# bistoyek21-ric/StrikeForce

Measured on AMD Instinct MI355X. Metric: env-steps/sec (whole node), 64x64 map x32 entities, higher is better.
Workload: dtype int32

## Files before the change

__graft_entry__.py:

```python
import os
import subprocess
import sys

ROOT = os.path.dirname(os.path.abspath(__file__))
for p in (ROOT, os.path.join(ROOT, "tests")):
    if p not in sys.path:
        sys.path.insert(0, p)


def build():
    from strikeforce_amd import build as b
    b.build()
    subprocess.check_call(["make", "-s", "-C", os.path.join(ROOT, "oracle"), "libsf_oracle.so"])
    subprocess.check_call(["make", "-s", "-C", os.path.join(ROOT, "oracle"), "ref"])
    subprocess.check_call(["make", "-s", "-C", os.path.join(ROOT, "tests", "emu"), "libsf_emu.so"])
    subprocess.check_call(["make", "-s", "-C", os.path.join(ROOT, "tests", "fixed_shape_emu"), "libsf_emu_fixed.so"])
    subprocess.check_call([sys.executable, "-B", os.path.join(ROOT, "tests", "obs_flavour.py")], stdout=subprocess.DEVNULL)
    import strikeforce_amd
    from strikeforce_amd import env
    lib = env.load_library()
    from strikeforce_amd import policy
    missing = [n for n in env.EXPORTS + policy.EXPORTS if not hasattr(lib, n)]
    if missing:
        raise RuntimeError("libstrikeforce_amd.so lacks %s" % missing)


def smoke():
    import numpy as np
    from oracle_lib import ArenaDump, Oracle, diff_dumps
    from strikeforce_amd import config, env

    w = config.baseline_workload("C1", arenas=4, device=0)
    o, g = Oracle(w), env.ArenaBatch(w)
    tb, sr = w.seeds()
    o.reset(tb, sr), g.reset(tb, sr)
    cmds, _ = config.bench_commands(4, 1, 40)
    for s in range(40):
        o.step(cmds[s]), g.step(cmds[s])
    for a in range(4):
        d = diff_dumps(o.dump(a).as_dict(), ArenaDump(*g.dump_raw(a)).as_dict())
        if d:
            raise AssertionError("smoke: arena %d differs from the oracle: %s" % (a, d))
    x, y = o.observe(), g.observe()
    ulp = np.abs(x.view(np.int32).astype(np.int64) - y.view(np.int32).astype(np.int64)).max()
    if ulp > 1:
        raise AssertionError("smoke: observation differs by %d ulp" % ulp)
    print("smoke ok: 4 arenas x 40 steps bit-exact, observation max ulp diff %d" % ulp)
    import ctypes as C
    import json
    import ref_cases
    gold = json.load(open(os.path.join(ROOT, "tests", "golden", "ref_traj.json")))["cases"]["C1"]
    wr = ref_cases.GOLDEN_CASES["C1"][0]()
    gr = env.ArenaBatch(wr)
    gr.reset((C.c_uint64 * 1)(gold["tb"]), (C.c_uint64 * 1)(gold["serial"]))
    rc, _ = config.bench_commands(1, 1, 60, seed0=gold["command_seed"])
    for s in range(60):
        if "%016x" % int(gr.digest()[0]) != gold["digests"][s]:
            raise AssertionError("smoke: state after %d steps differs from the reference's own" % s)
        gr.step(rc[s])
    print("smoke ok: 60 steps of configs[0] reproduce the reference's own per-step digests")
    import torch
    sys.path.insert(0, os.path.join(ROOT, "oracle"))
    import policy_ref
    from strikeforce_amd import policy
    params = policy.init_parameters(seed=1)
    pb = policy.PolicyBatch(params, 4)
    d_obs = torch.from_numpy(y.reshape(4, 32, 31, 31)).cuda()
    d_probs = torch.zeros((4, 9), device="cuda")
    d_value = torch.zeros(4, device="cuda")
    pb.forward(d_obs.data_ptr(), 4, d_probs.data_ptr(), d_value.data_ptr())
    pb.synchronize()
    h0 = np.zeros((2, 4, 160), dtype=np.float32)
    a0 = np.eye(9, dtype=np.float32)[[0] * 4]
    probs, value, _ = policy_ref.forward_batched(params, y.reshape(4, 32, 31, 31), h0, a0)
    err = float(np.max(np.abs(d_probs.cpu().numpy() - probs) / probs))
    if err > 5e-5 or np.max(np.abs(d_value.cpu().numpy() - value)) > 5e-5:
        raise AssertionError("smoke: policy network differs from the reference by %.3g" % err)
    print("smoke ok: policy forward for 4 agents, max relative error %.2g" % err)


if __name__ == "__main__":
    build()
    if "--smoke" in sys.argv:
        smoke()
```

strikeforce_amd/csrc/sf_api.hip:

```cpp
#include <hip/hip_runtime.h>

#include <dlfcn.h>

#include <cstddef>

#include <new>
#include <utility>
#include <vector>

#include "wave_gfx950.hpp"
#include "sf_core.hpp"
#include "sf_obs.hpp"
#include "sf_obs_kernels.hpp"
#include "sf_host.hpp"

namespace sf {

#ifdef SF_DIAG_STAMPS
__device__ uint32_t sf_diag_buffer[16 * 65536];
__device__ unsigned long long sf_diag_times[4 * 65536];
#endif

template <int NB, bool HP, bool BM, bool ZL>
__global__ __launch_bounds__(64) void k_reset(Params p, const uint64_t *tb, const uint64_t *serial) {
  extern __shared__ __attribute__((aligned(2048))) uint8_t lds[];
  Core<WaveGfx950, NB, HP, BM, ZL>::reset_body(lds, p, (int)blockIdx.x, tb, serial);
}

template <int NB, bool HP, bool BM, bool ZL, bool LOG>
__global__ __launch_bounds__(64) void k_step(Params p, const uint8_t *cmds, int k) {
  extern __shared__ __attribute__((aligned(2048))) uint8_t lds[];
  const int a = p.perm ? (int)gptr(p.perm)[blockIdx.x] : (int)blockIdx.x;
#ifdef SF_DIAG_STAMPS
  if (threadIdx.x == 0) sf_diag_times[4 * blockIdx.x] = __builtin_amdgcn_s_memrealtime();
#endif
  Core<WaveGfx950, NB, HP, BM, ZL>::template step_body_t<LOG>(lds, p, a, cmds, k);
#ifdef SF_DIAG_STAMPS
  __builtin_amdgcn_s_waitcnt(0);
  if (threadIdx.x == 0) sf_diag_times[4 * blockIdx.x + 3] = __builtin_amdgcn_s_memrealtime();
#endif
}

template <class SH>
__global__ __launch_bounds__(64) void k_step_fixed(Params p, const uint8_t *cmds, int k) {
  extern __shared__ __attribute__((aligned(2048))) uint8_t lds[];
  const int a = p.perm ? (int)gptr(p.perm)[blockIdx.x] : (int)blockIdx.x;
#ifdef SF_DIAG_STAMPS
  if (threadIdx.x == 0) sf_diag_times[4 * blockIdx.x] = __builtin_amdgcn_s_memrealtime();
#endif
  Core<WaveGfx950, SH::NB, false, true, false, SH>::template step_body_t<false>(lds, p, a, cmds, k);
#ifdef SF_DIAG_STAMPS
  __builtin_amdgcn_s_waitcnt(0);
  if (threadIdx.x == 0) sf_diag_times[4 * blockIdx.x + 3] = __builtin_amdgcn_s_memrealtime();
#endif
}

__global__ __launch_bounds__(1024) void k_rank(Params p, uint32_t *perm) {
  __shared__ uint32_t hist[72];
  const int t = (int)threadIdx.x;
  if (t < 72) hist[t] = 0u;
  __syncthreads();
  auto cls_of = [&](int a) {
    const uint32_t n = (uint32_t)gptr(p.scal)[(size_t)a * SC_WORDS + SC_LOAD];
    return 64u - (n > 64u ? 64u : n);
  };
  for (int a = t; a < p.A; a += 1024) atomicAdd(&hist[cls_of(a)], 1u);
  __syncthreads();
  if (t == 0) {
    uint32_t run = 0;
    for (int c = 0; c < 65; ++c) {
      const uint32_t n = hist[c];
      hist[c] = run;
      run += n;
    }
  }
  __syncthreads();
  for (int a = t; a < p.A; a += 1024) {
    uint32_t pos = atomicAdd(&hist[cls_of(a)], 1u);
    if ((pos >> 10) & 1u) {
      const uint32_t base = pos & ~1023u, len = (uint32_t)p.A - base < 1024u ? (uint32_t)p.A - base : 1024u;
      pos = base + (len - 1u - (pos - base));
    }
    gptr(perm)[pos] = (uint32_t)a;
  }
}

template <int NB, bool HP, bool BM, bool ZL>
__global__ __launch_bounds__(64) void k_step_half(Params p, const uint8_t *cmds, int phase) {
  extern __shared__ __attribute__((aligned(2048))) uint8_t lds[];
  Core<WaveGfx950, NB, HP, BM, ZL>::step_half_body(lds, p, (int)blockIdx.x, cmds, phase);
}

__global__ void k_agent_alive(Params p, uint8_t *out) {
  const int i = (int)(blockIdx.x * blockDim.x + threadIdx.x);
  if (i >= p.A * p.n_agents) return;
  const int a = i / p.n_agents, g = i % p.n_agents;
  const uint32_t fl = gptr(p.hum)[((size_t)HW_FLAGS * (size_t)p.A + (size_t)a) * (size_t)p.H + (size_t)g];
  gptr(out)[i] = (uint8_t)((fl & (HF_ALIVE | HF_CTRL)) == (HF_ALIVE | HF_CTRL));
}

__global__ void k_done(Params p, uint8_t *out) {
  const int i = (int)(blockIdx.x * blockDim.x + threadIdx.x);
  if (i >= p.A * p.n_agents) return;
  const SF_GLOBAL int32_t *sc = gptr(p.scal) + (size_t)(i / p.n_agents) * SC_WORDS;
  gptr(out)[i] = (uint8_t)(p.auto_reset ? sc[SC_ENDED] : sc[SC_DONE]);
}

__global__ __launch_bounds__(64) void k_ep_late(Params p, int after_reset) {
  Core<WaveGfx950, 1>::ep_log_late(p, (int)blockIdx.x, after_reset != 0);
}

__global__ __launch_bounds__(64) void k_replay_fetch(Params p, Replay r, int mode) {
  Core<WaveGfx950, 1>::replay_fetch(p, r, (int)blockIdx.x, mode);
}

__global__ __launch_bounds__(1024) void k_ep_plan(const int32_t *scal, int32_t *cursor, int A, int depth, int max_records,
                                                  int32_t *plan, int32_t *counts) {
  __shared__ int wsum[16];
  __shared__ int lost_sum;
  const int t = (int)threadIdx.x, lane = t & 63, w = t >> 6;
  const int chunk = (A + 1023) / 1024;
  const int a0 = min(t * chunk, A), a1 = min(a0 + chunk, A);
  int kept = 0, lost = 0;
#pragma unroll 4
  for (int a = a0; a < a1; ++a) {
    const int pend = max(gptr(scal)[(size_t)a * SC_WORDS + SC_EPISODES] - gptr(cursor)[a], 0);
    kept += min(pend, depth), lost += pend - min(pend, depth);
  }
  const int x = wave_scan_incl(kept, lane);
#pragma unroll
  for (int d = 32; d; d >>= 1) lost += __shfl_xor(lost, d, 64);
  if (t == 0) lost_sum = 0;
  if (lane == 63) wsum[w] = x;
// ... 587 lines not shown
```

strikeforce_amd/csrc/sf_core.hpp:

```cpp
#pragma once
#include "../../include/strikeforce.h"
#include "sf_types.hpp"

#if defined(SF_EXP_FAKE_DRAWS) && !defined(SF_EXPERIMENT_BUILD)
#error "SF_EXP_FAKE_DRAWS makes draw() return wrong numbers on purpose (tools/experiments/r03_rows): timing builds only, together with -DSF_EXPERIMENT_BUILD"
#endif

namespace sf {

enum { SH_WALL, SH_HUMAN, SH_ZOMBIE, SH_PUP, SH_PDN, SH_BULLET, SH_CHEST, SH_POUT, SH_EMPTY };
enum { LIM_PORTAL = 1000, LIM_BLOCK = 1100 };

#define SF_SHAPE(f) (SH::FIXED ? SH::f(p) : p.f)
template <class W, int NB, bool HBM_PLANE = false, bool BITMAPS = !HBM_PLANE, bool ZL = false, class SH = RuntimeShape>
struct Core {
  using V = typename W::V;
  using P = typename W::P;

  struct Arena {
    V hpos, hfl, hhp, hst, hmd, hk, hdm, hef, hc01, hc23, ht01, ht23, hbpk, hcmd;
    V zpos, zhp, zmd;
    uint32_t *zl;
    uint32_t zcap;
    uint32_t zwn;
    uint32_t zwhi;
    uint32_t *pl;
    uint32_t pwn, pwhi;
    V ba[NB], bd[NB], bb[NB], bc[NB];
    V ppos;
    V rl, rus, rseed;
    V rl2, rseed2;
    uint32_t warm;
    uint32_t wrate;
    const uint32_t *xt;
    const uint32_t *ht;
    uint32_t *bm;
    V la;
    V la2;
    uint32_t la2_ok;
    int32_t frame, kills, tkills, loot, chests, steps, episodes, done, outcome, ended;
    uint32_t jomle;
    uint32_t tb_lo, tb_hi, sr_lo, sr_hi;
    uint32_t dirty;
    uint32_t pd01, pd23, pd45;
#ifdef SF_DIAG_STAMPS
    V dacc;
    uint32_t dlast;
#endif
  };

  static constexpr uint32_t RL_ZERO = 0x10000u;
  static SF_DEV V mod65537_v(V x) {
    const V t = (x & 0xffffu) - (x >> 16);
    return W::minu(t, t + 65537u);
  }
  static SF_DEV V pow3_v(const uint32_t *xt, V m, P pred) {
    return mod65537_v(W::lds_u32(xt, m & 255u, pred) * W::lds_u32(xt + 256, m >> 8, pred));
  }

  template <bool WANT_OUT>
  static SF_DEV V draw_core(V &rl, const V &rus, const V &rseed, uint32_t &jomle, const uint32_t *xt, const Params &p) {
    const P tap = W::ltu(W::lane(), 18u) & ((rl & RL_ZERO) == 0u);
    const V pw = pow3_v(xt, (rl * rseed) & 0xffffu, tap);
    const V sum = W::sum18_row1(W::select(tap, rus * pw, V(0u))) + 1u;
    V t = mod65537_v(sum);
    t = W::select(t == 0u, V(1u), t);
    jomle += 1u;
    const uint32_t e = jomle & 0xffffu;
    const V lg = W::gload_u16(p.logt, t + (uint32_t)LOGT_OFF, W::all());
    const V lnew = (lg * e) & 0xffffu;
    rl = W::select(W::lane() == 17u, lnew, W::shl1(rl));
    if (WANT_OUT) return pow3_v(xt, lnew, W::all()) & 1023u;
    return V(0u);
  }
  static constexpr uint32_t SUM_BIAS_LANE = 63489u + 11u * 65537u;
  static_assert((32ull * SUM_BIAS_LANE) % 65537ull == 1ull, "the lanes' bias must add up to the generator's +1");
  static_assert(SUM_BIAS_LANE % 2u == 0u, "it is also a byte offset into a table of 16-bit entries");
  static_assert(16ull * SUM_BIAS_LANE > 16ull * 10ull * 65536ull, "a row's partial sum must stay positive");
  static_assert((32ull * SUM_BIAS_LANE + 18ull * 10ull * 65535ull) >> 16 < (unsigned long long)LOGT_OFF, "index below the table");
  static SF_DEV const uint16_t *log_base(const Params &p) { return p.logt + LOGT_OFF - (int)(SUM_BIAS_LANE / 2u); }
  static SF_DEV V issue_offset(const uint32_t *xt, V rl, V rseed, V rus, V &d) {
    const V m = W::mul24(rl, rseed);
    const V pr = W::pow_bytes(xt, m);
    d = (pr & 0xffffu) - (pr >> 16);
    return W::rng_reduce(d, rus, V(SUM_BIAS_LANE));
  }
  static SF_DEV uint32_t draw_issue(Arena &S, const Params &p) {
    V d;
    S.la = W::gload_u16_at(log_base(p), issue_offset(S.xt, S.rl, S.rseed, S.rus, d));
    W::rng_prio_end();
    const int32_t o = (int32_t)W::readlane(d, 18u);
    return (uint32_t)(o + ((o >> 31) & 65537)) & 1023u;
  }
  static SF_DEV uint32_t draw(Arena &S, const uint8_t *, const Params &p) {
#ifdef SF_EXP_FAKE_DRAWS
    S.jomle = S.jomle * 1664525u + 1013904223u;
    return (W::readlane(S.rl, (S.jomle >> 26) & 31u) ^ (S.jomle >> 16)) & 1023u;
#endif
    SF_PROF(PH_RNG);
    S.jomle += 1u;
    if constexpr (W::FUSED_ROUND) {
      uint32_t out;
      const V off = W::rng_round(S.rl, S.jomle, S.la, S.rseed, S.rus, V(SUM_BIAS_LANE), S.xt, out);
      S.la = W::gload_u16_at(log_base(p), off);
      return out;
    }
    S.rl = W::rng_commit(S.rl, S.jomle, S.la);
    return draw_issue(S, p);
  }

  static SF_DEV void seed_digits(V &digits, uint64_t x, uint32_t lane18 = 0u) {
    digits = V(0u);
    W::setlane(digits, 18u, lane18);
    for (int i = 0; i < 18; ++i) {
      W::setlane(digits, (uint32_t)i, (uint32_t)(x % 10u) + 1u);
      x /= 10u;
    }
  }
  static SF_DEV void srand_(Arena &S, const uint8_t *lds, const Params &p, uint64_t tb, uint64_t us) {
    S.rl = V(RL_ZERO);
    seed_digits(S.rus, us);
    seed_digits(S.rseed, tb, 1u);
    S.jomle = 18u;
    (void)lds;
    for (int i = 0; i < 1024; ++i) draw_core<false>(S.rl, S.rus, S.rseed, S.jomle, S.xt, p);
    draw_issue(S, p);
  }
  static SF_DEV void prewarm_issue(Arena &S, const Params &p) {
    V d;
    S.la2 = W::gload_u16_at(log_base(p), issue_offset(S.xt, S.rl2, S.rseed2, S.rus, d));
    S.la2_ok = 1u;
  }
// ... 1397 lines not shown
    }
    if (!W::uload_i32(sc + SC_ENDED)) return;
    const uint32_t ep = (uint32_t)W::uload_i32(sc + SC_EPISODES) - 1u;
    uint64_t tb = ((uint64_t)(uint32_t)W::uload_i32(sc + SC_TB_HI) << 32) | (uint32_t)W::uload_i32(sc + SC_TB_LO);
    if (SF_SHAPE(auto_reset)) tb -= (uint64_t)(uint32_t)p.reseed;
    const uint32_t *res = (const uint32_t *)p.results + (size_t)a * (size_t)SF_SHAPE(n_agents) * 8u;
    const uint32_t frame = (uint32_t)W::uload_i32((const int32_t *)res + 6), outcome = (uint32_t)W::uload_i32((const int32_t *)res + 7);
    V h = V((uint32_t)a);
    W::setlane(h, 1u, ep);
    W::setlane(h, 2u, (uint32_t)tb), W::setlane(h, 3u, (uint32_t)(tb >> 32));
    W::setlane(h, 4u, (uint32_t)W::uload_i32(sc + SC_SR_LO)), W::setlane(h, 5u, (uint32_t)W::uload_i32(sc + SC_SR_HI));
    W::setlane(h, 6u, (frame - 1u) / 2u), W::setlane(h, 7u, outcome);
    const V r = V(((uint32_t)a * depth + (ep & (depth - 1u))) * rw);
    W::gstore(ring, r + W::lane(), h, W::ltu(W::lane(), (uint32_t)EP_HDR_WORDS));
    const uint32_t n = 8u * (uint32_t)SF_SHAPE(n_agents);
    for (uint32_t i = 0u; i < n; i += 64u) {
      const P in = W::ltu(W::lane() + i, n);
      W::gstore(ring, r + (uint32_t)EP_HDR_WORDS + W::lane() + i, W::gload(res, W::lane() + i, in), in);
    }
  }

  static SF_DEV void replay_fetch(const Params &p, const Replay &r, int a, int mode) {
    int32_t *const st = r.status + (size_t)a * RP_WORDS;
    int32_t *const sc = p.scal + (size_t)a * SC_WORDS;
    const int32_t state = W::uload_i32(st + RP_STATE);
    const uint32_t cur = (uint32_t)W::uload_i32(st + RP_CURSOR);
    const uint32_t o0 = (uint32_t)W::uload_i32((const int32_t *)r.off + a), o1 = (uint32_t)W::uload_i32((const int32_t *)r.off + a + 1);
    const uint32_t len = o1 - o0;
    const int32_t done = W::uload_i32(sc + SC_DONE);
    const P ag = W::ltu(W::lane(), (uint32_t)SF_SHAPE(n_agents));
    const V row = W::lane() + (uint32_t)a * (uint32_t)SF_SHAPE(n_agents);
    const P me = W::lane() == (uint32_t)SF_SHAPE(ind);
    if (mode == 0) {
      bool go = false;
      if (state == SF_REPLAY_RUNNING && done) {
        W::ustore_i32(st + RP_STATE, SF_REPLAY_GAME_ENDED);
      } else if ((state == SF_REPLAY_RUNNING || state == SF_REPLAY_TRUNCATED) && !done) {
        if (state == SF_REPLAY_TRUNCATED || cur == len) {
          W::ustore_i32(sc + SC_DONE, 1), W::ustore_i32(sc + SC_OUTCOME, SF_SAMPLE_END);
          if (state == SF_REPLAY_RUNNING) W::ustore_i32(st + RP_STATE, SF_REPLAY_SAMPLE_ENDED);
        } else {
          go = true;
        }
      }
      const P first = go ? me : W::frombits(0ull);
      const V tok = W::gload_u8(r.streams, V(o0 + cur), first);
      W::gstore_u8(r.cmd, row, W::select(first, tok, V((uint32_t)'+')), ag);
      W::gstore_u8(r.taken, row, tok, ag);
      if (go) {
        W::ustore_i32(st + RP_CURSOR, (int32_t)(cur + 1u));
        W::ustore_i32(st + RP_ITER, W::uload_i32(st + RP_ITER) + 1);
      }
      return;
    }
    if (state != SF_REPLAY_RUNNING || done) return;
    const V fl = W::gload(p.hum, W::lane() + ((uint32_t)HW_FLAGS * (uint32_t)p.A + (uint32_t)a) * (uint32_t)SF_SHAPE(H), ag);
    const P takes = ag & !me & ((fl & (HF_ALIVE | HF_CTRL)) == (HF_ALIVE | HF_CTRL));
    const uint64_t bal = W::ballot(takes);
    const V line = V(cur) + W::rank_below(bal);
    const P have = takes & W::ltu(line, V(len));
    const V tok = W::gload_u8(r.streams, line + o0, have);
    W::gstore_u8(r.cmd, row, tok, have);
    W::gstore_u8(r.taken, row, tok, have);
    const uint32_t want = (uint32_t)W::popc64(bal), left = len - cur, got = want < left ? want : left;
    W::ustore_i32(st + RP_CURSOR, (int32_t)(cur + got));
    if (got < want) W::ustore_i32(st + RP_STATE, SF_REPLAY_TRUNCATED);
  }

  template <bool LOG = false>
  static SF_DEV void loop_top(Arena &S, uint8_t *lds, const Params &p, int a) {
    SF_PROF(PH_TOP);
    spawns(S, lds, p);
    const int out = check_end(S, p);
    if (out != SF_RUNNING) {
      S.done = 1, S.outcome = out;
      latch_results<LOG>(S, p, a);
    }
  }

  static SF_DEV void reset_state(Arena &S, uint8_t *lds, const Params &p, uint64_t tb, uint64_t serial, bool adopt) {
    S.frame = S.kills = S.tkills = S.loot = S.chests = S.steps = 0;
    S.done = 0, S.outcome = SF_RUNNING;
    S.tb_lo = (uint32_t)tb, S.tb_hi = (uint32_t)(tb >> 32), S.sr_lo = (uint32_t)serial, S.sr_hi = (uint32_t)(serial >> 32);
    S.hpos = V(POS_NONE), S.hfl = V(0u), S.hhp = V(0u), S.hst = V(0u), S.hmd = V(0u), S.hk = V(0u), S.hdm = V(0u);
    S.hef = V(0u), S.hc01 = V(0u), S.hc23 = V(0u), S.ht01 = V(0u), S.ht23 = V(0u), S.hbpk = V(0u);
    S.hcmd = V((uint32_t)'+');
    S.zpos = V(0u), S.zhp = V(0u), S.zmd = V(0u);
    if constexpr (ZL) S.zwn = 0u;
#pragma unroll
    for (int j = 0; j < NB; ++j) S.ba[j] = V(0u), S.bd[j] = V(0u), S.bb[j] = V(0u), S.bc[j] = V(0u);
    if constexpr (ZL) {
      S.ppos = V(0u);
      S.pwn = (uint32_t)p.pw0;
      for (uint32_t j = 0; j < S.pwn; ++j) {
        const V sl = W::lane() + 64u * j;
        W::lds_store_u32(S.pl + 64u * j, W::lane(), W::gload(p.map_exits, sl, W::ltu(sl, (uint32_t)p.P)), W::all());
      }
      if (S.pwhi < S.pwn) S.pwhi = S.pwn;
    } else {
      S.ppos = W::gload(p.map_exits, W::lane(), W::ltu(W::lane(), (uint32_t)p.P));
    }
    W::copy_g2l(lds, p.map_flags, (uint32_t)SF_SHAPE(cells_pad));
    S.dirty = 1u;
    if (adopt) {
      prewarm(S, lds, p, 1024u);
      S.rl = S.rl2, S.rseed = S.rseed2, S.jomle = 18u + 1024u;
      draw_issue(S, p);
    } else {
      srand_(S, lds, p, tb, serial);
    }
    if (SF_SHAPE(auto_reset)) {
      seed_digits(S.rseed2, tb + (uint64_t)(uint32_t)p.reseed, 1u);
      S.rl2 = V(RL_ZERO);
      S.warm = 0u, S.la2_ok = 0u;
    }
    const int count = SF_SHAPE(mode) == SF_MODE_BATTLE ? SF_SHAPE(n_agents) : (SF_SHAPE(mode) == SF_MODE_SQUAD ? 10 : 1);
    SF_NOUNROLL for (int i = 0; i < count; ++i) {
      int prof = 0, team = 1;
      uint32_t q = pos_pack(0, 1, 1), fl = HF_CTRL;
      if (SF_SHAPE(mode) == SF_MODE_BATTLE) {
        q = POS_NONE, team = p.tab->teams[i], fl = HF_CTRL | (i != SF_SHAPE(ind) ? HF_REMOTE : 0u);
      } else if (SF_SHAPE(mode) == SF_MODE_SQUAD) {
        prof = i ? 1 : 0;
        team = i < 5 ? 1 : 2;
        q = i == 0 ? pos_pack(0, 3, 1) : pos_pack(i < 5 ? 0 : p.squad_floor, 1, i + 1);
        fl = (i == 0 || i < SF_SHAPE(n_agents)) ? HF_CTRL : 0u;
      }
      human_make(S, p, (uint32_t)i, prof, q, 1, team, fl, (SF_SHAPE(mode) == SF_MODE_BATTLE && p.npc_block > 1) ? i : 0);
    }
    if (SF_SHAPE(mode) == SF_MODE_BATTLE) {
      S.hfl = S.hfl & ~HF_OCC;
      SF_NOUNROLL for (int i = 0; i < SF_SHAPE(n_agents); ++i) {
        const uint32_t way = draw(S, lds, p) % 4u + 1u;
        SF_NOUNROLL for (int guard = 0; guard < (1 << 20); ++guard) {
          const uint32_t q = draw_cell(S, lds, p);
          uint32_t fl;
          if (showit_q(S, lds, p, q, fl) == SH_EMPTY) {
            W::setlane(S.hpos, (uint32_t)i, q);
            W::setlane(S.hfl, (uint32_t)i, ((W::readlane(S.hfl, (uint32_t)i) & ~HF_WAY_MASK) | way) | HF_OCC);
            break;
          }
        }
      }
    }
  }

  template <int PHASE = 0, bool LOG = false>
  static SF_DEV void step(Arena &S, uint8_t *lds, const Params &p, int a) {
    if (S.done) return;
    SF_STAMP(S, 0);
    uint32_t rest = 0u;
    SF_NOUNROLL for (int half = (PHASE == 2 ? 1 : 0); half < (PHASE == 1 ? 1 : 2); ++half) {
      const uint32_t j0 = S.jomle;
      if (half == 0) {
        zombie_action(S, lds, p);
        SF_STAMP(S, 1);
      } else {
        human_action(S, lds, p, a);
        SF_STAMP(S, 3);
      }
      const uint32_t j1 = S.jomle;
      if (half == 0) {
        portal_damage(S, lds, p);
        SF_STAMP(S, 2);
      }
      if (SF_SHAPE(auto_reset)) prewarm(S, lds, p, S.wrate);
      SF_STAMP(S, 4);
      update_tmp(S, lds, p, a);
      SF_STAMP(S, 5);
      hits(S, p);
      SF_STAMP(S, 6);
      ++S.frame;
      if (SF_SHAPE(auto_reset)) prewarm(S, lds, p, S.wrate);
      SF_STAMP(S, 4);
      const uint32_t j2 = S.jomle;
      update_bull(S, lds, p);
      SF_STAMP(S, 7);
      const uint32_t w = ((j1 - j0) & 0xffffu) | ((S.jomle - j2) << 16);
      rest += j2 - j1;
      if (half == 0)
        S.pd01 = w;
      else
        S.pd23 = w;
    }
    if (PHASE == 1) return;
    ++S.steps;
    SF_NOUNROLL for (int pass = 0; pass < 2; ++pass) {
      const uint32_t j3 = S.jomle;
      loop_top<LOG>(S, lds, p, a);
      if (pass == 0) S.pd45 = ((S.jomle - j3) & 0xffffu) | (rest << 16);
      if (!S.done || pass == 1) break;
      if (S.ended < 255) ++S.ended;
      ++S.episodes;
      if (!SF_SHAPE(auto_reset)) break;
      const uint64_t tb = (((uint64_t)S.tb_hi << 32) | S.tb_lo) + (uint64_t)(uint32_t)p.reseed;
      const uint64_t sr = ((uint64_t)S.sr_hi << 32) | S.sr_lo;
      const int32_t ep = S.episodes;
      reset_state(S, lds, p, tb, sr, true);
      S.episodes = ep;
      ++S.frame;
    }
    SF_STAMP(S, 8);
  }

  static SF_DEV void load(Arena &S, uint8_t *lds, const Params &p, int a, bool copy_plane = true) {
    const V ln = W::lane();
    const size_t AH = (size_t)p.A * (size_t)SF_SHAPE(H), AZ = (size_t)p.A * (size_t)SF_SHAPE(Z), AB = (size_t)p.A * (size_t)SF_SHAPE(B);
    {
      const P in = W::ltu(ln, (uint32_t)SF_SHAPE(H));
      const uint32_t *h = p.hum + (size_t)a * (size_t)SF_SHAPE(H);
      S.hpos = W::gload(h + HW_POS * AH, ln, in), S.hfl = W::gload(h + HW_FLAGS * AH, ln, in);
      S.hhp = W::gload(h + HW_HP * AH, ln, in), S.hst = W::gload(h + HW_STAMINA * AH, ln, in);
      S.hmd = W::gload(h + HW_MINDAMAGE * AH, ln, in), S.hk = W::gload(h + HW_KILLS * AH, ln, in);
      S.hdm = W::gload(h + HW_DAMAGE * AH, ln, in), S.hef = W::gload(h + HW_EFFECT * AH, ln, in);
      S.hc01 = W::gload(h + HW_CONS01 * AH, ln, in), S.hc23 = W::gload(h + HW_CONS23 * AH, ln, in);
      S.ht01 = W::gload(h + HW_THR01 * AH, ln, in), S.ht23 = W::gload(h + HW_THR23 * AH, ln, in);
      S.hbpk = W::gload(h + HW_BPK * AH, ln, in);
      S.hcmd = V((uint32_t)'+');
    }
    if constexpr (ZL) {
      S.zpos = V(0u), S.zhp = V(0u), S.zmd = V(0u);
      const uint32_t *z = p.zom + (size_t)a * (size_t)SF_SHAPE(Z);
      S.zwn = (uint32_t)W::uload_i32(p.scal + (size_t)a * SC_WORDS + SC_ZWN);
      if (S.zwn > (uint32_t)zw_for(SF_SHAPE(Z))) S.zwn = (uint32_t)zw_for(SF_SHAPE(Z));
      S.zwhi = S.zwn;
      for (uint32_t j = 0; j < S.zwn; ++j) {
        const V sl = ln + 64u * j;
        const P in = W::ltu(sl, (uint32_t)SF_SHAPE(Z));
        zl_put(S, ZW_POS, j, W::gload(z + ZW_POS * AZ, sl, in), W::all());
        zl_put(S, ZW_HP, j, W::gload(z + ZW_HP * AZ, sl, in), W::all());
        zl_put(S, ZW_MINDAMAGE, j, W::gload(z + ZW_MINDAMAGE * AZ, sl, in), W::all());
      }
    } else {
      const P in = W::ltu(ln, (uint32_t)SF_SHAPE(Z));
      const uint32_t *z = p.zom + (size_t)a * (size_t)SF_SHAPE(Z);
      S.zpos = W::gload(z + ZW_POS * AZ, ln, in), S.zhp = W::gload(z + ZW_HP * AZ, ln, in);
      S.zmd = W::gload(z + ZW_MINDAMAGE * AZ, ln, in);
    }
#pragma unroll
    for (int j = 0; j < NB; ++j) {
      const V sl = ln + (uint32_t)(64 * j);
      const P in = W::ltu(sl, (uint32_t)SF_SHAPE(B));
      const uint32_t *b = p.bul + (size_t)a * (size_t)SF_SHAPE(B);
      S.ba[j] = W::gload(b + BW_A * AB, sl, in), S.bd[j] = W::gload(b + BW_DAMAGE * AB, sl, in);
      S.bb[j] = W::gload(b + BW_B * AB, sl, in), S.bc[j] = W::gload(b + BW_C * AB, sl, in);
    }
    if constexpr (ZL) {
      S.ppos = V(0u);
      S.pwn = (uint32_t)W::uload_i32(p.scal + (size_t)a * SC_WORDS + SC_PWN);
      if (S.pwn > (uint32_t)zw_for(p.P)) S.pwn = (uint32_t)zw_for(p.P);
      S.pwhi = S.pwn;
      for (uint32_t j = 0; j < S.pwn; ++j) {
        const V sl = ln + 64u * j;
        W::lds_store_u32(S.pl + 64u * j, ln, W::gload(p.por + (size_t)a * (size_t)p.P, sl, W::ltu(sl, (uint32_t)p.P)), W::all());
      }
    } else {
      S.ppos = W::gload(p.por + (size_t)a * (size_t)p.P, ln, W::ltu(ln, (uint32_t)p.P));
    }
    {
      const P in = W::ltu(ln, 18u);
      const V rw = W::gload(p.rng + (size_t)a * RNG_WORDS, ln, in);
      const V val = rw & 0xfffffu;
      S.rus = (rw >> 20) & 15u, S.rseed = W::select(ln == 18u, V(1u), (rw >> 24) & 15u);
        const P nz = in & (val != 0u);
      S.rl = W::select(nz, W::gload_u16(p.logt, val + (uint32_t)LOGT_OFF, nz), V(RL_ZERO));
      const V rw2 = W::gload(p.rng2 + (size_t)a * RNG_WORDS, ln, in);
      S.rl2 = rw2 & 0x1ffffu, S.rseed2 = W::select(ln == 18u, V(1u), rw2 >> 24);
    }
    const V sc = W::gload((const uint32_t *)p.scal + (size_t)a * SC_WORDS, ln, W::ltu(ln, (uint32_t)SC_WORDS));
    S.frame = (int32_t)W::readlane(sc, SC_FRAME), S.kills = (int32_t)W::readlane(sc, SC_KILLS);
    S.tkills = (int32_t)W::readlane(sc, SC_TKILLS), S.loot = (int32_t)W::readlane(sc, SC_LOOT);
    S.chests = (int32_t)W::readlane(sc, SC_CHESTS), S.jomle = W::readlane(sc, SC_JOMLE);
    S.steps = (int32_t)W::readlane(sc, SC_STEPS), S.episodes = (int32_t)W::readlane(sc, SC_EPISODES);
    S.done = (int32_t)W::readlane(sc, SC_DONE), S.outcome = (int32_t)W::readlane(sc, SC_OUTCOME);
    S.ended = (int32_t)W::readlane(sc, SC_ENDED);
    S.tb_lo = W::readlane(sc, SC_TB_LO), S.tb_hi = W::readlane(sc, SC_TB_HI);
    S.sr_lo = W::readlane(sc, SC_SR_LO), S.sr_hi = W::readlane(sc, SC_SR_HI);
    S.warm = W::readlane(sc, SC_WARM);
    S.pd01 = W::readlane(sc, SC_PD01), S.pd23 = W::readlane(sc, SC_PD23), S.pd45 = W::readlane(sc, SC_PD45);
    if (!HBM_PLANE && copy_plane) W::copy_g2l(lds, p.flags + (size_t)a * (size_t)SF_SHAPE(cells_pad), (uint32_t)SF_SHAPE(cells_pad));
    S.dirty = 0u;
    if (copy_plane) draw_issue(S, p);
  }

  static SF_DEV void store(const Arena &S, const uint8_t *lds, const Params &p, int a) {
// ... 72 lines not shown
      W::setlane(sc, SC_LOAD, (uint32_t)(W::popc64(W::ballot(((S.zpos & ZF_ALIVE) != 0u) & W::ltu(ln, (uint32_t)SF_SHAPE(Z)))) +
                                         W::popc64(W::ballot(((S.hfl & HF_ALIVE) != 0u) & W::ltu(ln, (uint32_t)SF_SHAPE(H))))));
    }
    W::gstore((uint32_t *)p.scal + (size_t)a * SC_WORDS, ln, sc, W::ltu(ln, (uint32_t)SC_WORDS));
    if (!HBM_PLANE && S.dirty) W::copy_l2g(p.flags + (size_t)a * (size_t)SF_SHAPE(cells_pad), lds, (uint32_t)SF_SHAPE(cells_pad));
  }

  static SF_DEV uint8_t *tables(Arena &S, uint8_t *lds, const Params &p, int a, bool copy = true) {
    uint8_t *tab = lds;
    if (copy) {
      W::copy_g2l(tab, reinterpret_cast<const uint8_t *>(p.exptab), (uint32_t)LDS_EXP_BYTES);
      W::copy_g2l(tab + LDS_EXP_BYTES, reinterpret_cast<const uint8_t *>(p.tab->hatab), (uint32_t)p.ht_bytes);
    }
    S.xt = reinterpret_cast<const uint32_t *>(tab);
    S.ht = reinterpret_cast<const uint32_t *>(tab + LDS_EXP_BYTES);
    S.bm = nullptr;
    if (BITMAPS) {
      S.bm = reinterpret_cast<uint32_t *>(lds + p.lds_tab + (HBM_PLANE ? 0 : SF_SHAPE(cells_pad)));
      W::lds_zero(S.bm, (uint32_t)(BM_COUNT * SF_SHAPE(bm_words)));
    }
    S.zl = nullptr, S.zcap = 0u, S.zwn = 0u, S.zwhi = 0u;
    S.pl = nullptr, S.pwn = 0u, S.pwhi = 0u;
    if constexpr (ZL) {
      S.zl = reinterpret_cast<uint32_t *>(lds + p.lds_tab + (HBM_PLANE ? 0 : SF_SHAPE(cells_pad)) + (BITMAPS ? BM_COUNT * 4 * SF_SHAPE(bm_words) : 0));
      S.zcap = 64u * (uint32_t)zw_for(SF_SHAPE(Z));
      S.pl = S.zl + ZW_WORDS * S.zcap;
    }
    S.la = V(0u);
    S.la2 = V(0u), S.la2_ok = 0u;
    return HBM_PLANE ? p.flags + (size_t)a * (size_t)SF_SHAPE(cells_pad) : lds + p.lds_tab;
  }

  static SF_DEV void reset_body(uint8_t *lds, const Params &p, int a, const uint64_t *tb, const uint64_t *serial) {
    Arena S;
    S.episodes = 0, S.ended = 0;
    S.pd01 = S.pd23 = S.pd45 = 0u;
    lds = tables(S, lds, p, a);
    S.rl2 = V(RL_ZERO), S.rseed2 = V(0u), S.warm = 0u, S.wrate = 1u;
    if constexpr (ZL) S.zwhi = (uint32_t)zw_for(SF_SHAPE(Z)), S.pwhi = (uint32_t)zw_for(p.P);
    reset_state(S, lds, p, tb[a], serial[a], false);
    ++S.frame;
    loop_top(S, lds, p, a);
    store(S, lds, p, a);
  }

  static SF_DEV void step_body(uint8_t *lds, const Params &p, int a, const uint8_t *cmds, int k) {
    if (p.tab->ep_ring)
      step_body_t<true>(lds, p, a, cmds, k);
    else
      step_body_t<false>(lds, p, a, cmds, k);
  }
  template <bool LOG>
  static SF_DEV void step_body_t(uint8_t *lds, const Params &p, int a, const uint8_t *cmds, int k) {
    Arena S;
    typename W::template G2L<LDS_EXP_BYTES / 1024> q_exp;
    typename W::template G2L<2> q_ht;
    typename W::template G2L<4> q_pl;
    uint8_t *const tab0 = lds;
    const uint32_t ht_n = (uint32_t)p.ht_bytes < 2048u ? (uint32_t)p.ht_bytes : 2048u;
    const uint32_t pl_n = HBM_PLANE ? 0u : ((uint32_t)SF_SHAPE(cells_pad) < 4096u ? (uint32_t)SF_SHAPE(cells_pad) : 4096u);
    const uint8_t *const pl_g = p.flags + (size_t)a * (size_t)SF_SHAPE(cells_pad);
    W::g2l_issue(q_exp, reinterpret_cast<const uint8_t *>(p.exptab), (uint32_t)LDS_EXP_BYTES);
    W::g2l_issue(q_ht, reinterpret_cast<const uint8_t *>(p.tab->hatab), ht_n);
    W::g2l_issue(q_pl, pl_g, pl_n);
    lds = tables(S, lds, p, a, false);
    load(S, lds, p, a, false);
    W::g2l_store(q_exp, tab0, (uint32_t)LDS_EXP_BYTES);
    W::g2l_store(q_ht, tab0 + LDS_EXP_BYTES, ht_n);
    if ((uint32_t)p.ht_bytes > ht_n)
      W::copy_g2l(tab0 + LDS_EXP_BYTES + ht_n, reinterpret_cast<const uint8_t *>(p.tab->hatab) + ht_n, (uint32_t)p.ht_bytes - ht_n);
    if (!HBM_PLANE) {
      W::g2l_store(q_pl, lds, pl_n);
      if ((uint32_t)SF_SHAPE(cells_pad) > pl_n) W::copy_g2l(lds + pl_n, pl_g + pl_n, (uint32_t)SF_SHAPE(cells_pad) - pl_n);
    }
    draw_issue(S, p);
    const P ag = W::ltu(W::lane(), (uint32_t)SF_SHAPE(n_agents));
    S.wrate = 4u;
    S.ended = 0;
    SF_STAMP_LOADED();
    SF_STAMP_BEGIN(S);
    for (int s = 0; s < k; ++s) {
      const uint8_t *c = cmds + ((size_t)s * (size_t)p.A + (size_t)a) * (size_t)SF_SHAPE(n_agents);
      S.hcmd = W::select(ag, W::gload_u8(c, W::lane(), ag), V((uint32_t)'+'));
      step<0, LOG>(S, lds, p, a);
    }
    SF_STAMP_END(S, a);
    SF_STAMP_STEPPED();
    store(S, lds, p, a);
  }

  static SF_DEV void step_half_body(uint8_t *lds, const Params &p, int a, const uint8_t *cmds, int phase) {
    Arena S;
    lds = tables(S, lds, p, a);
    load(S, lds, p, a);
    S.wrate = 4u;
    S.ended = 0;
    SF_STAMP_BEGIN(S);
    if (phase == 1) {
      S.hcmd = V((uint32_t)'+');
      step<1>(S, lds, p, a);
    } else {
      const P ag = W::ltu(W::lane(), (uint32_t)SF_SHAPE(n_agents));
      S.hcmd = W::select(ag, W::gload_u8(cmds + (size_t)a * (size_t)SF_SHAPE(n_agents), W::lane(), ag), V((uint32_t)'+'));
      step<2>(S, lds, p, a);
    }
    SF_STAMP_END(S, a);
    store(S, lds, p, a);
  }
};
#undef SF_SHAPE

}
```

strikeforce_amd/csrc/sf_types.hpp:

```cpp
#pragma once
#include <stddef.h>
#include <stdint.h>

#if defined(__HIPCC__)
#define SF_HD __host__ __device__
#else
#define SF_HD
#endif

namespace sf {

constexpr uint32_t POS_MASK = 0x3FFFFFu;
constexpr uint32_t POS_NONE = 0x3FFFFFu;
SF_HD inline uint32_t pos_pack(int f, int r, int c) {
  return ((uint32_t)f << 20) | ((uint32_t)r << 10) | (uint32_t)c;
}
SF_HD inline int pos_f(uint32_t p) { return (int)((p >> 20) & 3u); }
SF_HD inline int pos_r(uint32_t p) { return (int)((p >> 10) & 1023u); }
SF_HD inline int pos_c(uint32_t p) { return (int)(p & 1023u); }

enum { HW_POS = 0, HW_FLAGS, HW_HP, HW_STAMINA, HW_MINDAMAGE, HW_KILLS, HW_DAMAGE, HW_EFFECT, HW_CONS01, HW_CONS23,
       HW_THR01, HW_THR23, HW_BPK, HW_WORDS };
constexpr uint32_t HF_WAY_MASK = 7u;
constexpr int HF_TEAM_SH = 3;
// ... 58 lines not shown

enum { RP_STATE = 0, RP_CURSOR, RP_ITER, RP_PAD, RP_WORDS };
struct Replay {
  const uint8_t *streams;
  const uint32_t *off;
  int32_t *status;
  uint8_t *cmd;
  uint8_t *taken;
};

struct Params {
  int32_t A, F, N, M, cells, cells_pad;
  int32_t bm_words;
  int32_t H, Z, B, P, C;
  int32_t mode, level, n_agents, auto_reset, reseed, timer_lim, squad_floor;
  int32_t ind;
  int32_t npc_block;
  int32_t ht_bytes;
  int32_t lds_tab;
  int32_t pw0;
  const Tables *tab;
  uint32_t *hum;
  uint32_t *zom;
  uint32_t *bul;
  uint32_t *por;
  uint32_t *rng;
  uint32_t *rng2;
  int32_t *scal;
  int32_t *results;
  uint8_t *flags;
  int32_t *aux_dmg;
  int16_t *aux_pidx;
  const uint8_t *map_flags;
  const int16_t *map_pidx;
  const uint32_t *map_exits;
  const uint16_t *logt;
  const uint32_t *exptab;
  const uint32_t *perm;
};

constexpr int LOGT_OFF = 1024;
constexpr int LOGT_ENTRIES = LOGT_OFF + 65537;

constexpr int BM_COUNT = 3;
constexpr int bm_words_for(int cells);
inline bool use_bitmaps(int cells_pad) { return BM_COUNT * 4 * bm_words_for(cells_pad) <= 6 * 1024; }
constexpr int bm_words_for(int cells) { return ((cells + 31) / 32 + 3) & ~3; }

inline int nb_for(int B) { return (B + 63) / 64; }
SF_HD inline bool large_pools(int Z, int P) { return Z > 64 || P > 64; }
SF_HD inline int zw_for(int n) { return (n + 63) / 64; }
inline size_t zl_bytes_for(int Z, int P) {
  return large_pools(Z, P) ? 4u * 64u * ((size_t)ZW_WORDS * (size_t)zw_for(Z) + (size_t)zw_for(P)) : 0u;
}
constexpr int LDS_EXP_BYTES = 2048;
inline int lds_tab_for(int blocks) { return LDS_EXP_BYTES + ht_bytes_for(blocks); }
inline bool hbm_plane(int cells_pad);
inline size_t lds_zl_offset(int cells_pad, int lds_tab) {
  return (size_t)lds_tab + (hbm_plane(cells_pad) ? 0u : (size_t)cells_pad) +
         (use_bitmaps(cells_pad) ? (size_t)BM_COUNT * 4u * (size_t)bm_words_for(cells_pad) : 0u);
}
inline size_t lds_bytes_for(int cells_pad, int lds_tab, int Z, int P) {
  return lds_zl_offset(cells_pad, lds_tab) + zl_bytes_for(Z, P);
}
constexpr int LDS_PLANE_MAX = 12 * 1024;
inline bool hbm_plane(int cells_pad) { return cells_pad > LDS_PLANE_MAX; }

#define SF_SHAPE_FIELDS(X) X(F) X(N) X(M) X(cells) X(cells_pad) X(bm_words) X(H) X(Z) X(B) X(mode) X(level) X(n_agents) X(auto_reset) X(ind)
struct RuntimeShape {
  static constexpr bool FIXED = false;
#define SF_SHAPE_ACCESSOR(f) \
  static SF_HD int32_t f(const Params &p) { return p.f; }
  SF_SHAPE_FIELDS(SF_SHAPE_ACCESSOR)
#undef SF_SHAPE_ACCESSOR
};
template <int F_, int N_, int M_, int H_, int Z_, int B_, int MODE_, int LEVEL_, int N_AGENTS_, int AUTO_RESET_, int IND_>
struct FixedShape {
  static constexpr bool FIXED = true;
  struct Values {
    static constexpr int32_t F = F_, N = N_, M = M_, cells = F_ * N_ * M_, cells_pad = (cells + 15) & ~15,
                             bm_words = bm_words_for(cells_pad), H = H_, Z = Z_, B = B_, mode = MODE_, level = LEVEL_,
                             n_agents = N_AGENTS_, auto_reset = AUTO_RESET_, ind = IND_;
  };
  static_assert(Values::cells_pad <= LDS_PLANE_MAX && Z_ <= 64 && H_ <= 64 && B_ <= 256, "a fixed shape is an LDS-plane, register-pool shape");
  static constexpr int NB = (B_ + 63) / 64;
#define SF_SHAPE_ACCESSOR(f) \
  static SF_HD constexpr int32_t f(const Params &) { return Values::f; }
  SF_SHAPE_FIELDS(SF_SHAPE_ACCESSOR)
#undef SF_SHAPE_ACCESSOR
  static bool matches(const Params &p) {
#define SF_SHAPE_EQUAL(f) &&p.f == Values::f
    return !large_pools(p.Z, p.P) SF_SHAPE_FIELDS(SF_SHAPE_EQUAL);
#undef SF_SHAPE_EQUAL
  }
};
template <class... S>
struct ShapeList {};
using FixedShapes = ShapeList<
    FixedShape<1, 64, 64, 8, 24, 64, 1 , 1, 1, 1, 0>,
    FixedShape<1, 64, 64, 1, 16, 32, 0 , 1, 1, 1, 0>
    >;
inline int fixed_shape_of(const Params &, ShapeList<>, int = 0) { return -1; }
template <class S0, class... S>
inline int fixed_shape_of(const Params &p, ShapeList<S0, S...>, int first = 0) {
  return S0::matches(p) ? first : fixed_shape_of(p, ShapeList<S...>{}, first + 1);
}
template <class F>
inline int with_fixed_shape(int, ShapeList<>, int none, F &&) { return none; }
template <class F, class S0, class... S>
inline int with_fixed_shape(int index, ShapeList<S0, S...>, int none, F &&f) {
  return index == 0 ? f(S0{}) : with_fixed_shape(index - 1, ShapeList<S...>{}, none, f);
}

template <int NB_, bool HP_, bool BM_, bool ZL_>
struct KernelVariant {
  static constexpr int NB = NB_;
  static constexpr bool HP = HP_, BM = BM_, ZL = ZL_;
};
template <int NB, bool ZL, class F>
int with_plane_variant(const Params &p, F &&f) {
  if (!hbm_plane(p.cells_pad)) return f(KernelVariant<NB, false, true, ZL>{});
  if (use_bitmaps(p.cells_pad)) return f(KernelVariant<NB, true, true, ZL>{});
  return f(KernelVariant<NB, true, false, ZL>{});
}
template <class F>
int with_variant(const Params &p, int NB, F &&f) {
  if (large_pools(p.Z, p.P)) return with_plane_variant<4, true>(p, f);
  switch (NB) {
    case 1: return with_plane_variant<1, false>(p, f);
    case 2: return with_plane_variant<2, false>(p, f);
    case 3: return with_plane_variant<3, false>(p, f);
    default: return with_plane_variant<4, false>(p, f);
  }
}

}
```

Measured before the change: 234.2 million.

## Split fixed-shape step into single pass with rare restart path; add large fixed shape

For fixed-shape kernels, the per-step loop now runs a single loop_top pass and calls a separate restart routine only when an episode just ended. The goal is to keep the reset path out of the common step and let the compiler specialise it. The fixed-shape reset also zeroes registers through an opaque asm barrier, and fixed shapes gain HBM-plane and bitmap variants plus a 256x256 shape with a waves-per-EU hint. The restart ordering could diverge from the original two-pass semantics, which is why a new restart emulator test is added.

```diff
diff --git a/__graft_entry__.py b/__graft_entry__.py
--- a/__graft_entry__.py
+++ b/__graft_entry__.py
@@ -15,6 +15,7 @@
     subprocess.check_call(["make", "-s", "-C", os.path.join(ROOT, "oracle"), "ref"])
     subprocess.check_call(["make", "-s", "-C", os.path.join(ROOT, "tests", "emu"), "libsf_emu.so"])
     subprocess.check_call(["make", "-s", "-C", os.path.join(ROOT, "tests", "fixed_shape_emu"), "libsf_emu_fixed.so"])
+    subprocess.check_call(["make", "-s", "-C", os.path.join(ROOT, "tests", "restart_emu"), "libsf_emu_restart.so"])
     subprocess.check_call([sys.executable, "-B", os.path.join(ROOT, "tests", "obs_flavour.py")], stdout=subprocess.DEVNULL)
     import strikeforce_amd
     from strikeforce_amd import env
diff --git a/strikeforce_amd/csrc/sf_api.hip b/strikeforce_amd/csrc/sf_api.hip
--- a/strikeforce_amd/csrc/sf_api.hip
+++ b/strikeforce_amd/csrc/sf_api.hip
@@ -42,13 +42,13 @@
 }
 
 template <class SH>
-__global__ __launch_bounds__(64) void k_step_fixed(Params p, const uint8_t *cmds, int k) {
+__global__ __launch_bounds__(64) __attribute__((amdgpu_waves_per_eu(SH::HP ? 4 : 1))) void k_step_fixed(Params p, const uint8_t *cmds, int k) {
   extern __shared__ __attribute__((aligned(2048))) uint8_t lds[];
   const int a = p.perm ? (int)gptr(p.perm)[blockIdx.x] : (int)blockIdx.x;
 #ifdef SF_DIAG_STAMPS
   if (threadIdx.x == 0) sf_diag_times[4 * blockIdx.x] = __builtin_amdgcn_s_memrealtime();
 #endif
-  Core<WaveGfx950, SH::NB, false, true, false, SH>::template step_body_t<false>(lds, p, a, cmds, k);
+  Core<WaveGfx950, SH::NB, SH::HP, SH::BM, false, SH>::template step_body_t<false>(lds, p, a, cmds, k);
 #ifdef SF_DIAG_STAMPS
   __builtin_amdgcn_s_waitcnt(0);
   if (threadIdx.x == 0) sf_diag_times[4 * blockIdx.x + 3] = __builtin_amdgcn_s_memrealtime();
diff --git a/strikeforce_amd/csrc/sf_core.hpp b/strikeforce_amd/csrc/sf_core.hpp
--- a/strikeforce_amd/csrc/sf_core.hpp
+++ b/strikeforce_amd/csrc/sf_core.hpp
@@ -4,6 +4,10 @@
 
 #if defined(SF_EXP_FAKE_DRAWS) && !defined(SF_EXPERIMENT_BUILD)
 #error "SF_EXP_FAKE_DRAWS makes draw() return wrong numbers on purpose (tools/experiments/r03_rows): timing builds only, together with -DSF_EXPERIMENT_BUILD"
+#endif
+
+#if defined(SF_EXP_NO_RESTART) && !defined(SF_EXPERIMENT_BUILD)
+#error "SF_EXP_NO_RESTART leaves an arena whose episode ended standing still (tools/restart_ceiling.py): timing builds only, together with -DSF_EXPERIMENT_BUILD"
 #endif
 
 namespace sf {
@@ -48,6 +52,22 @@
     uint32_t dlast;
 #endif
   };
+
+  static SF_DEV void here(V &x) {
+#if defined(__HIP_DEVICE_COMPILE__)
+    asm volatile("" : "+v"(x));
+#else
+    (void)x;
+#endif
+  }
+  template <class T>
+  static SF_DEV void here(const T *&x) {
+#if defined(__HIP_DEVICE_COMPILE__)
+    asm volatile("" : "+s"(x));
+#else
+    (void)x;
+#endif
+  }
 
   static constexpr uint32_t RL_ZERO = 0x10000u;
   static SF_DEV V mod65537_v(V x) {
@@ -1611,6 +1631,16 @@
     S.frame = S.kills = S.tkills = S.loot = S.chests = S.steps = 0;
     S.done = 0, S.outcome = SF_RUNNING;
     S.tb_lo = (uint32_t)tb, S.tb_hi = (uint32_t)(tb >> 32), S.sr_lo = (uint32_t)serial, S.sr_hi = (uint32_t)(serial >> 32);
+    if constexpr (SH::FIXED) {
+      V z = V(0u);
+      here(z);
+      S.hpos = z | POS_NONE, S.hfl = z, S.hhp = z, S.hst = z, S.hmd = z, S.hk = z, S.hdm = z;
+      S.hef = z, S.hc01 = z, S.hc23 = z, S.ht01 = z, S.ht23 = z, S.hbpk = z;
+      S.hcmd = V((uint32_t)'+');
+      S.zpos = z, S.zhp = z, S.zmd = z;
+#pragma unroll
+      for (int j = 0; j < NB; ++j) S.ba[j] = z, S.bd[j] = z, S.bb[j] = z, S.bc[j] = z;
+    } else {
     S.hpos = V(POS_NONE), S.hfl = V(0u), S.hhp = V(0u), S.hst = V(0u), S.hmd = V(0u), S.hk = V(0u), S.hdm = V(0u);
     S.hef = V(0u), S.hc01 = V(0u), S.hc23 = V(0u), S.ht01 = V(0u), S.ht23 = V(0u), S.hbpk = V(0u);
     S.hcmd = V((uint32_t)'+');
@@ -1618,6 +1648,7 @@
     if constexpr (ZL) S.zwn = 0u;
 #pragma unroll
     for (int j = 0; j < NB; ++j) S.ba[j] = V(0u), S.bd[j] = V(0u), S.bb[j] = V(0u), S.bc[j] = V(0u);
+    }
     if constexpr (ZL) {
       S.ppos = V(0u);
       S.pwn = (uint32_t)p.pw0;
@@ -1674,7 +1705,7 @@
     }
   }
 
-  template <int PHASE = 0, bool LOG = false>
+  template <int PHASE = 0, bool LOG = false, bool SPLIT = false>
   static SF_DEV void step(Arena &S, uint8_t *lds, const Params &p, int a) {
     if (S.done) return;
     SF_STAMP(S, 0);
@@ -1714,6 +1745,13 @@
     }
     if (PHASE == 1) return;
     ++S.steps;
+    if constexpr (SPLIT) {
+      const uint32_t j3 = S.jomle;
+      loop_top<LOG>(S, lds, p, a);
+      S.pd45 = ((S.jomle - j3) & 0xffffu) | (rest << 16);
+      SF_STAMP(S, 8);
+      return;
+    }
     SF_NOUNROLL for (int pass = 0; pass < 2; ++pass) {
       const uint32_t j3 = S.jomle;
       loop_top<LOG>(S, lds, p, a);
@@ -1730,6 +1768,25 @@
       ++S.frame;
     }
     SF_STAMP(S, 8);
+  }
+
+  template <bool LOG>
+  static SF_DEV void restart(Arena &S, uint8_t *lds, const Params &p, int a) {
+    if (S.ended < 255) ++S.ended;
+    ++S.episodes;
+    if (!SF_SHAPE(auto_reset)) return;
+#ifdef SF_EXP_NO_RESTART
+    return;
+#endif
+    Params q = p;
+    here(q.map_exits), here(q.map_flags);
+    const uint64_t tb = (((uint64_t)S.tb_hi << 32) | S.tb_lo) + (uint64_t)(uint32_t)q.reseed;
+    const uint64_t sr = ((uint64_t)S.sr_hi << 32) | S.sr_lo;
+    const int32_t ep = S.episodes;
+    reset_state(S, lds, q, tb, sr, true);
+    S.episodes = ep;
+    ++S.frame;
+    loop_top<LOG>(S, lds, q, a);
   }
 
   static SF_DEV void load(Arena &S, uint8_t *lds, const Params &p, int a, bool copy_plane = true) {
@@ -1968,7 +2025,13 @@
     for (int s = 0; s < k; ++s) {
       const uint8_t *c = cmds + ((size_t)s * (size_t)p.A + (size_t)a) * (size_t)SF_SHAPE(n_agents);
       S.hcmd = W::select(ag, W::gload_u8(c, W::lane(), ag), V((uint32_t)'+'));
-      step<0, LOG>(S, lds, p, a);
+      if constexpr (SH::FIXED) {
+        const int32_t was_done = S.done;
+        step<0, LOG, true>(S, lds, p, a);
+        if (__builtin_expect(!was_done && S.done, 0)) restart<LOG>(S, lds, p, a);
+      } else {
+        step<0, LOG>(S, lds, p, a);
+      }
     }
     SF_STAMP_END(S, a);
     SF_STAMP_STEPPED();
diff --git a/strikeforce_amd/csrc/sf_types.hpp b/strikeforce_amd/csrc/sf_types.hpp
--- a/strikeforce_amd/csrc/sf_types.hpp
+++ b/strikeforce_amd/csrc/sf_types.hpp
@@ -164,8 +164,10 @@
                              bm_words = bm_words_for(cells_pad), H = H_, Z = Z_, B = B_, mode = MODE_, level = LEVEL_,
                              n_agents = N_AGENTS_, auto_reset = AUTO_RESET_, ind = IND_;
   };
-  static_assert(Values::cells_pad <= LDS_PLANE_MAX && Z_ <= 64 && H_ <= 64 && B_ <= 256, "a fixed shape is an LDS-plane, register-pool shape");
+  static_assert(Z_ <= 64 && H_ <= 64 && B_ <= 256, "a fixed shape is a register-pool shape");
   static constexpr int NB = (B_ + 63) / 64;
+  static constexpr bool HP = Values::cells_pad > LDS_PLANE_MAX;
+  static constexpr bool BM = BM_COUNT * 4 * Values::bm_words <= 6 * 1024;
 #define SF_SHAPE_ACCESSOR(f) \
   static SF_HD constexpr int32_t f(const Params &) { return Values::f; }
   SF_SHAPE_FIELDS(SF_SHAPE_ACCESSOR)
@@ -180,7 +182,8 @@
 struct ShapeList {};
 using FixedShapes = ShapeList<
     FixedShape<1, 64, 64, 8, 24, 64, 1 , 1, 1, 1, 0>,
-    FixedShape<1, 64, 64, 1, 16, 32, 0 , 1, 1, 1, 0>
+    FixedShape<1, 64, 64, 1, 16, 32, 0 , 1, 1, 1, 0>,
+    FixedShape<1, 256, 256, 8, 56, 128, 3 , 1, 8, 1, 0>
     >;
 inline int fixed_shape_of(const Params &, ShapeList<>, int = 0) { return -1; }
 template <class S0, class... S>
```

New measurement: 234.5 million, median of 5. Within noise of the previous version (+0.1%).
